# 2892931976/consensus-rs

Measured on AMD Instinct MI355X. Metric: BFT instance-rounds/sec (whole node), N=64 f=21, 1/2/4/8 GPUs; bit-exact, higher is better.
Workload: dtype u64

## Files before the change

### __graft_entry__.py

```python
import os
import subprocess
import sys

ROOT = os.path.dirname(os.path.abspath(__file__))
PKG = os.path.join(ROOT, "consensus-rs_amd")


def _make(path, *targets):
    jobs = str(min(8, os.cpu_count() or 1))
    subprocess.check_call(["make", "-s", "-j", jobs, "-C", path, *targets])


def build() -> None:
    env_arch = os.environ.get("PYTORCH_ROCM_ARCH", "gfx950")
    assert "gfx950" in env_arch, "this framework targets gfx950 only"
    _make(PKG)
    _make(os.path.join(ROOT, "oracle"))
    sys.path.insert(0, os.path.join(ROOT, "tests"))
    import emu_lib
    emu_lib.build()
    import sig_lib
    sig_lib.build()
    import wire_lib
    wire_lib.build()
    import trace_lib
    trace_lib.build()
    import twins_lib
    twins_lib.build()
    import audit_lib
    audit_lib.build()
    import ledger_lib
    ledger_lib.build()
    import archive_lib
    archive_lib.build()
    import accuse_lib
    accuse_lib.build()
    import timeline_lib
    timeline_lib.build()
    import rollcall_lib
    rollcall_lib.build()
    sys.path.insert(0, PKG)
    import bftsim
    from bftsim import runtime
    runtime.lib()
    from bftsim import sig, wire
    sig.lib()
    wire.lib()


def smoke() -> None:
    sys.path.insert(0, PKG)
    sys.path.insert(0, os.path.join(ROOT, "tests"))
    import numpy as np
    import torch
    from bftsim.configs import cfg3
    from bftsim.runtime import Simulator
    import oracle_lib as O
    assert torch.cuda.is_available(), "smoke() needs an MI355X"
    cfg = cfg3(heights=10)
    sim = Simulator(cfg, device=0)
    got = sim.run(0, 4)
    sim.close()
    ref = O.run(cfg, 0, 4)
    for k in ("committed_height", "flags", "ticks", "views", "round", "proposer", "variant",
              "time_tick", "block_hash"):
        if not np.array_equal(got[k], ref[k]):
            raise AssertionError(f"smoke: HIP result differs from the oracle in {k}")
    assert (got["committed_height"] == 10).all()
    print("smoke ok:", int(got["views"].sum()), "instance-rounds bit-exact vs oracle")


if __name__ == "__main__":
    build()
    if len(sys.argv) > 1 and sys.argv[1] == "smoke":
        smoke()
```

### consensus-rs_amd/csrc/bft_common.h

```cpp
#pragma once
#include <stdint.h>

#if defined(__HIPCC__)
#include <hip/hip_runtime.h>
#define BFT_FN __host__ __device__ inline
#else
#define BFT_FN inline
#endif

namespace bft {

struct Params {
    uint32_t n;
    uint32_t seg;
    uint32_t heights;
    uint32_t hcap;
    uint32_t max_ticks;
    uint32_t block_period;
    uint64_t genesis_time;
    uint64_t seed;
    uint32_t thr16;
    uint32_t byz_count;
    uint32_t crash_thr32;
    uint32_t crash_on;
// ... 643 lines not shown
    return (uint32_t)((((uint64_t)hi << 32) | lo) >> (8u * r));
#endif
}
BFT_FN uint32_t splice_blocks(uint32_t len_p, uint32_t len_s) { return (len_p + len_s + 136u) / 136u; }
BFT_FN uint32_t splice_word(const uint32_t* sx, uint32_t r, const uint32_t* pw, uint32_t w, uint32_t nb) {
    uint32_t v = align_bytes(sx[w + 1u], sx[w], r);
    if (w < 2u * PFX_WORDS) v |= pw[w];
    if (w == 34u * nb - 1u) v ^= 0x80000000u;
    return v;
}
BFT_FN uint32_t header_words(uint64_t* wb, const uint32_t prev[8], const uint8_t* addr20, uint64_t seed,
                             uint32_t inst, uint32_t h, uint32_t prop, uint32_t var, uint64_t time) {
    HdrWriter w(wb);
    header_fields(w, prev, addr20, seed, inst, h, prop, var, time);
    return w.finish();
}
BFT_FN uint32_t header_raw(uint64_t* wb, const uint32_t prev[8], const uint8_t* addr20, uint64_t seed,
                           uint32_t inst, uint32_t h, uint32_t prop, uint32_t var, uint64_t time) {
    HdrWriter w(wb);
    header_fields(w, prev, addr20, seed, inst, h, prop, var, time);
    const uint32_t len = 8u * w.wi + w.fill;
    if (w.fill) wb[w.wi] = w.acc;
    return len;
}

BFT_FN void lane_block_hash(uint8_t* buf, const uint32_t prev[8], const uint8_t* addr20, uint64_t seed,
                            uint32_t inst, uint32_t h, uint32_t prop, uint32_t var, uint64_t time,
                            uint32_t out[8]) {
    uint64_t* wb = (uint64_t*)buf;
    const uint32_t nb = header_words(wb, prev, addr20, seed, inst, h, prop, var, time);
    uint64_t a[25];
#pragma unroll
    for (int i = 0; i < 25; ++i) a[i] = 0;
#pragma unroll 1
    for (uint32_t blk = 0; blk < nb; ++blk) {
        const uint64_t* w = wb + 17u * blk;
#pragma unroll
        for (int i = 0; i < 17; ++i) a[i] ^= w[i];
        keccak_f1600(a);
    }
#pragma unroll
    for (int i = 0; i < 4; ++i) { out[2 * i] = (uint32_t)a[i]; out[2 * i + 1] = (uint32_t)(a[i] >> 32); }
}

BFT_FN uint32_t header_prefix_regs(const uint32_t prev[8], const PfxSel* tbl, uint32_t pw[2 * PFX_WORDS]) {
    uint64_t wv[PFX_WORDS];
#pragma unroll
    for (uint32_t k = 0; k < PFX_WORDS; ++k) wv[k] = 0;
    uint64_t acc = 0x2000dc9dull;
    uint32_t fill = 4, wi = 0;
#pragma unroll
    for (uint32_t i = 0; i < 8; ++i) {
        const uint32_t w = prev[i];
        const uint32_t idx = ((((w >> 7) & 0x01010101u) * 0x10204080u) >> 28);
        const PfxSel sel = tbl[idx];
        const uint64_t v = (uint64_t)perm_bytes(0xccccccccu, w, sel.lo) | ((uint64_t)perm_bytes(0xccccccccu, w, sel.hi) << 32);
        const uint32_t n = 4u + (uint32_t)__builtin_popcount(idx);
        const uint32_t sh = 8u * fill, nf = fill + n;
        const uint64_t lo = acc | (v << sh);
#pragma unroll
        for (uint32_t k = (1u + i) / 2u; k <= i; ++k) wv[k] = wi == k ? lo : wv[k];
        const bool full = nf >= 8u;
        acc = full ? (sh ? v >> (64u - sh) : 0ull) : lo;
        wi += full ? 1u : 0u;
        fill = full ? nf - 8u : nf;
    }
#pragma unroll
    for (uint32_t k = 4; k < PFX_WORDS; ++k) wv[k] = wi == k ? acc : wv[k];
#pragma unroll
    for (uint32_t k = 0; k < PFX_WORDS; ++k) { pw[2 * k] = (uint32_t)wv[k]; pw[2 * k + 1] = (uint32_t)(wv[k] >> 32); }
    return 8u * wi + fill;
}

#if !defined(__HIP_DEVICE_COMPILE__)
inline void spliced_block_hash(const uint32_t* sfx, const uint32_t prev[8], uint32_t out[8]) {
    for (int i = 0; i < 8; ++i) out[i] = 0;
    uint32_t buf[SFX_BUF] = {};
    for (uint32_t i = 0; i < SFX_BODY_DW; ++i) buf[SFX_PAD + i] = sfx[i];
    uint64_t pfx[PFX_WORDS + 4], ref[PFX_WORDS];
    PfxSel tbl[16];
    for (uint32_t i = 0; i < 16; ++i) tbl[i] = pfx_sel(i);
    const uint32_t lp = header_prefix_perm(pfx, prev, tbl);
    if (header_prefix(ref, prev) != lp) return;
    for (uint32_t i = 0; i < PFX_WORDS; ++i) if (ref[i] != pfx[i]) return;
    uint32_t pr[2 * PFX_WORDS];
    if (header_prefix_regs(prev, tbl, pr) != lp) return;
    for (uint32_t i = 0; i < PFX_WORDS; ++i) if (pr[2 * i] != (uint32_t)ref[i] || pr[2 * i + 1] != (uint32_t)(ref[i] >> 32)) return;
    uint32_t pw[2 * PFX_WORDS];
    for (uint32_t i = 0; i < PFX_WORDS; ++i) { pw[2 * i] = (uint32_t)pfx[i]; pw[2 * i + 1] = (uint32_t)(pfx[i] >> 32); }
    const uint32_t c = 72u - lp, nb = splice_blocks(lp, sfx[SFX_LEN_DW]);
    const uint32_t* sx = buf + (c >> 2);
    uint64_t a[25] = {};
    for (uint32_t blk = 0; blk < nb; ++blk) {
        for (uint32_t i = 0; i < 17; ++i) {
            const uint32_t w = 34u * blk + 2u * i;
            a[i] ^= (uint64_t)splice_word(sx, c & 3u, pw, w, nb) | ((uint64_t)splice_word(sx, c & 3u, pw, w + 1u, nb) << 32);
        }
        keccak_f1600(a);
    }
    for (int i = 0; i < 4; ++i) { out[2 * i] = (uint32_t)a[i]; out[2 * i + 1] = (uint32_t)(a[i] >> 32); }
}
#endif

template <uint32_t STRIDE = 1>
BFT_FN uint64_t byz_mask64(uint64_t seed, uint32_t inst, uint32_t f, uint8_t* perm) {
    auto at = [&](uint32_t i) -> uint8_t& { return perm[(i >> 2) * 4u * STRIDE + (i & 3u)]; };
    for (uint32_t i = 0; i < 64u; ++i) at(i) = (uint8_t)i;
    uint64_t mask = 0;
    if (f > 64u) f = 64u;
    for (uint32_t i = 0; i < f; ++i) {
        uint32_t w[4];
        philox(seed, inst, i, 0, DOM_BYZ, w);
        const uint32_t j = i + w[0] % (64u - i);
        const uint8_t t = at(i); at(i) = at(j); at(j) = t;
        mask |= 1ull << at(i);
    }
    return mask;
}
constexpr uint32_t SPEC_VALID = 0x80000000u;
BFT_FN bool spec_block64(uint64_t seed, uint32_t inst, uint32_t x, uint64_t byz, uint32_t tip_w0, uint32_t& j,
                         uint32_t& var) {
    j = tip_w0 & 63u;
    uint64_t v1m = 0;
    if ((byz >> j) & 1ull) {
        uint32_t w[4];
        philox(seed, inst, x, 0, DOM_SPLIT, w);
        v1m = ((uint64_t)w[0] | ((uint64_t)w[1] << 32)) & ~(1ull << j);
    }
    const uint64_t hon = ~byz;
    const bool k0 = __builtin_popcountll(byz | (hon & ~v1m)) > 42, k1 = __builtin_popcountll(byz | (hon & v1m)) > 42;
    var = k1 ? 1u : 0u;
    return k0 != k1;
}
BFT_FN uint32_t spec_word(uint32_t j, uint32_t var, uint32_t seed_next) { return SPEC_VALID | j | (var << 8) | (seed_next << 16); }

BFT_FN uint32_t seed_from_hash(const uint8_t* h, uint32_t n, bool le = false) {
    if (le) {
        uint64_t v = 0;
        for (int i = 7; i >= 0; --i) v = (v << 8) | h[i];
        return (uint32_t)(v % n);
    }
    uint64_t be = 0;
    for (int i = 0; i < 8; ++i) be = (be << 8) | h[i];
    uint64_t a = be % n;
    uint64_t t = (0xffffffffffffffffull % n + 1ull) % n;
    return (uint32_t)((a * t) % n);
}
BFT_FN uint32_t seed_from_words(uint32_t w0, uint32_t w1, uint32_t n, bool le) {
    uint8_t hb[8];
    for (int q = 0; q < 4; ++q) { hb[q] = (uint8_t)(w0 >> (8 * q)); hb[4 + q] = (uint8_t)(w1 >> (8 * q)); }
    return seed_from_hash(hb, n, le);
}

}
```

### consensus-rs_amd/csrc/bft_hip.h

```cpp
#pragma once
#include <hip/hip_runtime.h>

#include "../../include/bftsim.h"
#include "bft_common.h"
#include "bft_wave.h"

namespace bft {

struct WaveHip {
    __device__ void init(uint8_t*) {}
    __device__ static uint32_t lane() { return __lane_id(); }
    __device__ static uint64_t ballot(bool p) { return __builtin_amdgcn_ballot_w64(p); }
    __device__ static uint32_t shfl_xor(uint32_t v, int m) { return (uint32_t)__shfl_xor((int)v, m, 64); }
    __device__ static uint32_t shfl(uint32_t v, uint32_t src) { return (uint32_t)__shfl((int)v, (int)src, 64); }
    template <int N> __device__ static uint32_t row_shl(uint32_t v) {
        return (uint32_t)__builtin_amdgcn_mov_dpp((int)v, 0x100 + N, 0xF, 0xF, true);
    }
    template <int N> __device__ static uint32_t row_shr(uint32_t v) {
        return (uint32_t)__builtin_amdgcn_mov_dpp((int)v, 0x110 + N, 0xF, 0xF, true);
    }
    __device__ static uint32_t bperm(uint32_t addr, uint32_t v) { return (uint32_t)__builtin_amdgcn_ds_bpermute((int)addr, (int)v); }
    __device__ static uint32_t pair_swap(uint32_t v) { return (uint32_t)__builtin_amdgcn_mov_dpp((int)v, 0xB1, 0xF, 0xF, false); }
    template <uint32_t N> __device__ static uint32_t rotl_pair(uint32_t mine, uint32_t other) {
        if constexpr (N == 0) return mine;
// ... 60 lines not shown
    __device__ static void gadd64(uint64_t* p, uint64_t v) { atomicAdd((unsigned long long*)p, (unsigned long long)v); }
};

template <int NW>
struct GroupHip {
    uint64_t* slot;
    uint32_t par;
    __device__ void init(uint8_t* p) { slot = (uint64_t*)p; par = 0; }
    __device__ uint32_t lane() const { return threadIdx.x; }
    __device__ uint64_t* cur() const { return slot + par * 4u; }
    __device__ Bits<NW> ballot(bool p) {
        uint64_t b = __ballot(p);
        uint64_t* s = cur();
        if (__lane_id() == 0) s[threadIdx.x >> 6] = b;
        __syncthreads();
        Bits<NW> r;
#pragma unroll
        for (int k = 0; k < NW; ++k) r.w[k] = s[k];
        par ^= 1u;
        return r;
    }
    __device__ uint32_t bcast(uint32_t v, uint32_t j) {
        uint64_t* s = cur();
        if (threadIdx.x == j) s[0] = v;
        __syncthreads();
        uint32_t r = (uint32_t)s[0];
        par ^= 1u;
        return r;
    }
    __device__ uint32_t grp_max(uint32_t v) {
        for (int m = 1; m < 64; m <<= 1) { uint32_t o = (uint32_t)__shfl_xor((int)v, m, 64); v = v > o ? v : o; }
        uint64_t* s = cur();
        if (__lane_id() == 0) s[threadIdx.x >> 6] = v;
        __syncthreads();
        uint32_t r = 0;
#pragma unroll
        for (int k = 0; k < NW; ++k) r = (uint32_t)s[k] > r ? (uint32_t)s[k] : r;
        par ^= 1u;
        return r;
    }
    __device__ uint32_t grp_or(uint32_t v) {
        for (int m = 1; m < 64; m <<= 1) v |= (uint32_t)__shfl_xor((int)v, m, 64);
        uint64_t* s = cur();
        if (__lane_id() == 0) s[threadIdx.x >> 6] = v;
        __syncthreads();
        uint32_t r = 0;
#pragma unroll
        for (int k = 0; k < NW; ++k) r |= (uint32_t)s[k];
        par ^= 1u;
        return r;
    }
    __device__ uint64_t grp_sum64(uint32_t v32) {
        uint64_t v = v32;
        for (int m = 1; m < 64; m <<= 1) {
            uint32_t lo = (uint32_t)__shfl_xor((int)(uint32_t)v, m, 64), hi = (uint32_t)__shfl_xor((int)(uint32_t)(v >> 32), m, 64);
            v += (uint64_t)lo | ((uint64_t)hi << 32);
        }
        uint64_t* s = cur();
        if (__lane_id() == 0) s[threadIdx.x >> 6] = v;
        __syncthreads();
        uint64_t r = 0;
#pragma unroll
        for (int k = 0; k < NW; ++k) r += s[k];
        par ^= 1u;
        return r;
    }
    __device__ void sync() { __syncthreads(); par ^= 1u; }
    __device__ uint64_t* big() const { return slot + 8 + par * 64u; }
    template <int K> __device__ void ballot_k(const bool (&p)[K], Bits<NW> (&out)[K]) {
        static_assert(K * NW <= 64, "batched ballot area");
        uint64_t* s = big();
        uint64_t b[K];
#pragma unroll
        for (int k = 0; k < K; ++k) b[k] = __ballot(p[k]);
        if (__lane_id() == 0) {
#pragma unroll
            for (int k = 0; k < K; ++k) s[k * NW + (threadIdx.x >> 6)] = b[k];
        }
        __syncthreads();
#pragma unroll
        for (int k = 0; k < K; ++k)
#pragma unroll
            for (int w = 0; w < NW; ++w) out[k].w[w] = s[k * NW + w];
        par ^= 1u;
    }
    __device__ uint64_t* summary() const { return slot + 8 + 2u * 64u; }
    template <int K> __device__ void ballot_k_store(const bool (&p)[K], uint64_t* dst) {
        uint64_t b[K];
#pragma unroll
        for (int k = 0; k < K; ++k) b[k] = __ballot(p[k]);
        if (__lane_id() == 0) {
#pragma unroll
            for (int k = 0; k < K; ++k) dst[k * NW + (threadIdx.x >> 6)] = b[k];
        }
        __syncthreads();
        par ^= 1u;
    }
    template <int K> __device__ void gather_k(const bool (&wr)[K], const uint32_t (&v)[K], uint32_t (&out)[K]) {
        static_assert(K <= 128, "batched gather area");
        uint32_t* s = (uint32_t*)big();
#pragma unroll
        for (int k = 0; k < K; ++k)
            if (wr[k]) s[k] = v[k];
        __syncthreads();
#pragma unroll
        for (int k = 0; k < K; ++k) out[k] = s[k];
        par ^= 1u;
    }
    __device__ static uint64_t clock() { return __builtin_amdgcn_s_memtime(); }
    __device__ static uint32_t gload(const uint32_t* p) {
        return __hip_atomic_load(p, __ATOMIC_RELAXED, __HIP_MEMORY_SCOPE_AGENT);
    }
    __device__ static void gstore(uint32_t* p, uint32_t v) {
        __hip_atomic_store(p, v, __ATOMIC_RELAXED, __HIP_MEMORY_SCOPE_AGENT);
    }
    __device__ static void gstore4(uint32_t* p, uint32_t a, uint32_t b, uint32_t c, uint32_t d) {
        *(uint4*)p = make_uint4(a, b, c, d);
    }
    __device__ static void lds_add(uint32_t* p, uint32_t v) { atomicAdd(p, v); }
    __device__ static void gadd64(uint64_t* p, uint64_t v) { atomicAdd((unsigned long long*)p, (unsigned long long)v); }
};

hipError_t launch_general_0_0(uint32_t seg, dim3 grid, size_t lds, hipStream_t s, const Params& p);
hipError_t launch_general_0_1(uint32_t seg, dim3 grid, size_t lds, hipStream_t s, const Params& p);
hipError_t launch_general_1_0(uint32_t seg, dim3 grid, size_t lds, hipStream_t s, const Params& p);
hipError_t launch_general_1_1(uint32_t seg, dim3 grid, size_t lds, hipStream_t s, const Params& p);
inline hipError_t launch_general(bool need_seed, bool ext, uint32_t seg, dim3 grid, size_t lds, hipStream_t s,
                                 const Params& p) {
    if (need_seed) return ext ? launch_general_1_1(seg, grid, lds, s, p) : launch_general_1_0(seg, grid, lds, s, p);
    return ext ? launch_general_0_1(seg, grid, lds, s, p) : launch_general_0_0(seg, grid, lds, s, p);
}
hipError_t launch_fast(dim3 grid, hipStream_t s, const Params& p);
hipError_t launch_hash_suffix(uint32_t n, uint32_t x0, uint32_t rows, uint32_t* sfx, bool loop, hipStream_t s,
                              Params p);
constexpr uint32_t CHAIN_KERNEL_PAIR = 0, CHAIN_KERNEL_WAVE = 1, CHAIN_KERNEL_LANE = 2;
hipError_t launch_hash_chain(uint32_t n, uint32_t x0, uint32_t rows, uint32_t* sfx, uint32_t kind, hipStream_t s,
                             Params p);
constexpr uint32_t CHAIN_MAX_SETS = 32;
struct ChainSets {
    uint32_t count;
    const uint32_t* sfx[CHAIN_MAX_SETS];
    const uint32_t* ch[CHAIN_MAX_SETS];
    uint8_t* hash[CHAIN_MAX_SETS];
    uint32_t first[CHAIN_MAX_SETS];
    uint64_t* byz[CHAIN_MAX_SETS];
    uint32_t* bad[CHAIN_MAX_SETS];
    const uint32_t* rec[CHAIN_MAX_SETS];
    uint32_t* pred[CHAIN_MAX_SETS];
};
constexpr uint32_t CHAIN_RECORDED = 0;
constexpr uint32_t CHAIN_PREDICTED = 1;
constexpr uint32_t CHAIN_REPAIR = 2;
hipError_t launch_hash_chain_batch(uint32_t n, const ChainSets& cs, uint32_t kind, hipStream_t s, Params p);
hipError_t launch_spec_suffix(uint32_t n, const ChainSets& cs, hipStream_t s, const Params& p);
hipError_t launch_spec_verify(uint32_t n, const ChainSets& cs, hipStream_t s, const Params& p);
hipError_t launch_seed_chain(uint32_t n, hipStream_t s, const Params& p);
hipError_t launch_resume(dim3 grid, size_t lds, hipStream_t s, const Params& p);

}
```

### consensus-rs_amd/csrc/bftsim.hip

```cpp
#include <hip/hip_runtime.h>

#include <stdio.h>
#include <stdlib.h>
#include <string.h>

#include <dlfcn.h>
#include <unistd.h>
#include <rccl/rccl.h>
#include <hipcub/hipcub.hpp>

#include <mutex>
#include <string>
#include <utility>
#include <vector>

#include "bft_hip.h"
#include "bft_fast64.h"
#include "bft_crypto.h"
#include "bft_trace.h"
#include "bft_twins.h"
#include "bft_audit.h"
#include "bft_archive.h"
#include "bft_accuse.h"
#include "bft_timeline.h"
// ... 616 lines not shown
    use_set0_scratch(h);
    if (h->n_sets == 0) {
        (void)hipFree(h->d_ch); (void)hipFree(h->d_flags); (void)hipFree(h->d_ticks); (void)hipFree(h->d_views);
        (void)hipFree(h->d_rec); (void)hipFree(h->d_hash);
    }
    for (uint32_t k = 0; k < h->n_sets; ++k) {
        bftsim::RowSet& r = h->sets[k];
        (void)hipFree(r.ch); (void)hipFree(r.flags); (void)hipFree(r.ticks); (void)hipFree(r.views);
        (void)hipFree(r.rec); (void)hipFree(r.hash); (void)hipFree(r.sfx); (void)hipFree(r.spec);
        (void)hipFree(r.byz); (void)hipFree(r.bad); (void)hipFree(r.pred);
        if (k > 0) {
            (void)hipFree(r.hist); (void)hipFree(r.rcs); (void)hipFree(r.backlog); (void)hipFree(r.resume);
            (void)hipFree(r.save); (void)hipFree(r.resume_q);
        }
        r.ch = r.flags = r.ticks = nullptr; r.views = nullptr; r.rec = nullptr; r.hash = nullptr; r.sfx = nullptr;
        r.spec = nullptr; r.byz = nullptr; r.bad = nullptr; r.pred = nullptr;
        r.hist = nullptr; r.rcs = r.backlog = r.resume = r.save = r.resume_q = nullptr;
    }

    (void)hipFree(h->d_trace); (void)hipFree(h->d_tips); (void)hipFree(h->d_rcs);
    h->d_rcs = nullptr;
    (void)hipFree(h->d_backlog);
    h->d_backlog = nullptr;
    (void)hipFree(h->d_mlog); (void)hipFree(h->d_mlog_n);
    h->d_mlog = nullptr; h->d_mlog_n = nullptr;
    (void)hipFree(h->d_vsnap); (void)hipFree(h->d_votes); (void)hipFree(h->d_vsig); (void)hipFree(h->d_vhas);
    h->d_vsnap = nullptr; h->d_votes = nullptr; h->d_vsig = nullptr; h->d_vhas = nullptr; h->vsig_n = 0;
    h->backlog_bytes = 0;
    (void)hipFree(h->d_resume); (void)hipFree(h->d_save); (void)hipFree(h->d_resume_q);
    h->d_resume = nullptr; h->d_save = nullptr; h->d_resume_q = nullptr;
    for (uint32_t k = 0; k < bftsim::MAX_SETS; ++k) h->sets[k].busy = false;
    h->n_sets = 0;
    h->cur_set = 0;
    h->d_ch = h->d_flags = h->d_ticks = nullptr; h->d_views = nullptr;
    h->d_rec = nullptr; h->d_hash = nullptr; h->d_trace = nullptr; h->d_tips = nullptr;
    h->cap_inst = 0;
    h->n_req = 0;
    h->last_n = 0;
    h->last_first = 0;
}

static int flush_batch(bftsim* h, bool final = false);
static int sync_all(bftsim* h) {
    HIPCHECK(h, hipSetDevice(h->device));
    if (int rc = flush_batch(h, true)) return rc;
    HIPCHECK(h, hipStreamSynchronize(h->last_stream));
    for (uint32_t k = 0; k < bftsim::MAX_CS; ++k)
        if (h->cs[k]) HIPCHECK(h, hipStreamSynchronize(h->cs[k]));
    for (uint32_t k = 0; k < bftsim::MAX_HS; ++k)
        if (h->hstr[k]) HIPCHECK(h, hipStreamSynchronize(h->hstr[k]));
    return BFTSIM_OK;
}

#ifdef BFT_STAMPS
static uint64_t* g_stamps = nullptr;
static uint64_t g_stamp_waves = 0;
#endif

namespace {
struct Rccl {
    ncclResult_t (*get_id)(ncclUniqueId*) = nullptr;
    ncclResult_t (*init_rank)(ncclComm_t*, int, ncclUniqueId, int) = nullptr;
    ncclResult_t (*all_reduce)(const void*, void*, size_t, ncclDataType_t, ncclRedOp_t, ncclComm_t,
                               hipStream_t) = nullptr;
    ncclResult_t (*destroy)(ncclComm_t) = nullptr;
    const char* (*err)(ncclResult_t) = nullptr;
    bool ok = false;
    std::string why;
};
Rccl& rccl() {
    static Rccl r;
    static std::once_flag once;
    std::call_once(once, [] {
        void* lib = dlopen("librccl.so.1", RTLD_NOW | RTLD_GLOBAL);
        if (!lib) lib = dlopen("/opt/rocm/lib/librccl.so.1", RTLD_NOW | RTLD_GLOBAL);
        if (!lib) { r.why = std::string("dlopen librccl.so.1: ") + dlerror(); return; }
        r.get_id = (decltype(r.get_id))dlsym(lib, "ncclGetUniqueId");
        r.init_rank = (decltype(r.init_rank))dlsym(lib, "ncclCommInitRank");
        r.all_reduce = (decltype(r.all_reduce))dlsym(lib, "ncclAllReduce");
        r.destroy = (decltype(r.destroy))dlsym(lib, "ncclCommDestroy");
        r.err = (decltype(r.err))dlsym(lib, "ncclGetErrorString");
        r.ok = r.get_id && r.init_rank && r.all_reduce && r.destroy && r.err;
        if (!r.ok) r.why = "librccl.so.1 lacks an entry point";
    });
    return r;
}
struct StdoutToStderr {
    int saved;
    StdoutToStderr() {
        fflush(stdout);
        saved = dup(1);
        if (saved >= 0) dup2(2, 1);
    }
    ~StdoutToStderr() {
        fflush(stdout);
        if (saved >= 0) { dup2(saved, 1); close(saved); }
    }
};
void comm_destroy(ncclComm_t c) {
    if (rccl().ok) (void)rccl().destroy(c);
}

struct SigApi {
    int (*create)(int, void**) = nullptr;
    void (*destroy)(void*) = nullptr;
    const char* (*last_error)(const void*) = nullptr;
    int (*secret_to_address)(void*, const uint8_t*, uint64_t, uint8_t*, uint8_t*, uint8_t*, void*) = nullptr;
    int (*sign)(void*, const uint8_t*, const uint32_t*, const uint8_t*, uint64_t, uint8_t*, uint8_t*, void*) = nullptr;
    int (*recover)(void*, const uint8_t*, const uint8_t*, uint64_t, uint8_t*, uint8_t*, uint8_t*, void*) = nullptr;
    bool ok = false;
    std::string why;
};
void sig_api_anchor() {}
SigApi& sig_api() {
    static SigApi a;
    static std::once_flag once;
    std::call_once(once, [] {
        Dl_info di;
        std::string path = "libbftsig.so";
        if (dladdr((void*)&sig_api_anchor, &di) && di.dli_fname) {
            std::string self = di.dli_fname;
            size_t k = self.rfind('/');
            if (k != std::string::npos) path = self.substr(0, k + 1) + "libbftsig.so";
        }
        void* lib = dlopen(path.c_str(), RTLD_NOW | RTLD_GLOBAL);
        if (!lib) { a.why = std::string("dlopen ") + path + ": " + dlerror(); return; }
        a.create = (decltype(a.create))dlsym(lib, "bftsig_create");
        a.destroy = (decltype(a.destroy))dlsym(lib, "bftsig_destroy");
        a.last_error = (decltype(a.last_error))dlsym(lib, "bftsig_last_error");
        a.secret_to_address = (decltype(a.secret_to_address))dlsym(lib, "bftsig_secret_to_address");
        a.sign = (decltype(a.sign))dlsym(lib, "bftsig_sign");
        a.recover = (decltype(a.recover))dlsym(lib, "bftsig_recover");
        a.ok = a.create && a.destroy && a.last_error && a.secret_to_address && a.sign && a.recover;
        if (!a.ok) a.why = path + " lacks an entry point";
    });
    return a;
}
}

extern "C" {

#ifdef BFT_STAMPS
int bftsim_debug_stamps(uint64_t* out, uint32_t cap) {
    if (!out || cap == 0) return bft::NSTAMP;
    std::vector<uint64_t> v(g_stamp_waves * bft::NSTAMP);
    if (hipDeviceSynchronize() != hipSuccess) return -2;
    if (hipMemcpy(v.data(), g_stamps, v.size() * 8, hipMemcpyDeviceToHost) != hipSuccess) return -2;
    const uint32_t m = cap < (uint32_t)bft::NSTAMP ? cap : (uint32_t)bft::NSTAMP;
    for (uint32_t k = 0; k < m; ++k) out[k] = 0;
    for (uint64_t w = 0; w < g_stamp_waves; ++w)
        for (uint32_t k = 0; k < m; ++k) out[k] += v[w * bft::NSTAMP + k];
    return bft::NSTAMP;
}
#endif

uint32_t bftsim_two_thirds_majority(uint32_t n) { return (2u * n) / 3u; }
uint32_t bftsim_seed_from_hash(const uint8_t hash[32], uint32_t n) { return n ? bft::seed_from_hash(hash, n) : 0; }
uint32_t bftsim_seed_from_hash_order(const uint8_t hash[32], uint32_t n, uint32_t order) {
    return n ? bft::seed_from_hash(hash, n, order == BFTSIM_SEED_LE) : 0;
}
uint32_t bftsim_calc_proposer(const uint8_t prev_hash[32], uint32_t n, uint64_t round) {
    if (n == 0) return 0;
    return (uint32_t)(((uint64_t)bft::seed_from_hash(prev_hash, n) + round % n) % n);
}
void bftsim_keccak256(const uint8_t* data, size_t len, uint8_t out[32]) { host_keccak(data, len, out); }
void bftsim_genesis_hash(const bftsim_config* cfg, uint8_t out[32]) { host_genesis_hash(cfg, out); }
int bftsim_check_message(uint32_t code, uint64_t msg_height, uint64_t core_height, uint32_t state) {
    if (code < 1 || code > 4 || state < 1 || state > 4 || msg_height >= (1ull << 32) || core_height >= (1ull << 32))
        return BFTSIM_EINVAL;
    return bft::check_message_class((int)code, (uint32_t)msg_height, (uint32_t)core_height, state);
}
int bftsim_view_cmp(uint64_t h1, uint64_t r1, uint64_t h2, uint64_t r2) {
    if (h1 != h2) return h1 < h2 ? -1 : 1;
    if (r1 != r2) return r1 < r2 ? -1 : 1;
    return 0;
}

const char* bftsim_last_error(bftsim_t* h) { return h ? h->err.c_str() : "null handle"; }

int bftsim_create(const bftsim_config* cfg, int hip_device, bftsim_t** out) {
    if (!cfg || !out) return BFTSIM_EINVAL;
    *out = nullptr;
    if (cfg->n < 1 || cfg->n > 256) return BFTSIM_EUNSUPPORTED;
    if (cfg->heights < 1 || cfg->heights > (1u << 20) || cfg->max_ticks < 1 || cfg->max_ticks > (1u << 28) ||
        !cfg->addresses || cfg->phase_cap < 1 || cfg->phase_cap > 255 || cfg->block_period < 1)
        return BFTSIM_EINVAL;
    for (uint32_t i = 1; i < cfg->n; ++i)
        if (memcmp(cfg->addresses + 20 * (i - 1), cfg->addresses + 20 * i, 20) >= 0) return BFTSIM_EINVAL;
    if (cfg->seed_byte_order > BFTSIM_SEED_LE || cfg->header_encoding != BFTSIM_ENC_RMP_COMPACT ||
        cfg->backlog_mode > BFTSIM_BACKLOG_REPLAY || cfg->reserved != 0)
        return BFTSIM_EINVAL;
    bftsim* h = new bftsim();
    h->cfg = *cfg;
    h->addresses.assign(cfg->addresses, cfg->addresses + 20 * cfg->n);
    h->cfg.addresses = h->addresses.data();
    h->device = hip_device;
    host_genesis_hash(&h->cfg, h->genesis_hash);
    h->genesis_seed = bft::seed_from_hash(h->genesis_hash, cfg->n, cfg->seed_byte_order == BFTSIM_SEED_LE);
    h->seg = bft::segment_size(cfg->n);
    h->hcap = cfg->heights + 64;
    *out = h;
    hipError_t e = hipSetDevice(hip_device);
    if (e != hipSuccess) return fail(h, BFTSIM_EHIP, std::string("hipSetDevice: ") + hipGetErrorString(e));
    HIPCHECK(h, hipMalloc(&h->d_addr, 20 * cfg->n));
    HIPCHECK(h, hipMemcpy(h->d_addr, h->addresses.data(), 20 * cfg->n, hipMemcpyHostToDevice));
    HIPCHECK(h, hipMalloc(&h->d_ghash, 32));
    HIPCHECK(h, hipMemcpy(h->d_ghash, h->genesis_hash, 32, hipMemcpyHostToDevice));
    HIPCHECK(h, hipMalloc(&h->d_stats, 16 * sizeof(unsigned long long)));
    HIPCHECK(h, hipMalloc(&h->d_hist, bft::HIST_BINS * sizeof(uint64_t)));
    for (uint32_t i = 0; i < bftsim::RING; ++i) {
        HIPCHECK(h, hipEventCreate(&h->ring[i].c0)); HIPCHECK(h, hipEventCreate(&h->ring[i].c1));
        HIPCHECK(h, hipEventCreate(&h->ring[i].h0)); HIPCHECK(h, hipEventCreate(&h->ring[i].h1));
        HIPCHECK(h, hipEventCreateWithFlags(&h->ring[i].sx, hipEventDisableTiming));
    }
    for (uint32_t i = 0; i < bftsim::MAX_SETS; ++i)
        HIPCHECK(h, hipEventCreateWithFlags(&h->sets[i].done, hipEventDisableTiming));
    return BFTSIM_OK;
}

void bftsim_destroy(bftsim_t* h) {
    if (!h) return;
    (void)hipSetDevice(h->device);
    free_bufs(h);
    (void)hipFree(h->d_addr); (void)hipFree(h->d_ghash); (void)hipFree(h->d_stats); (void)hipFree(h->d_hist);
    (void)hipFree(h->d_red);
    (void)hipFree(h->d_evict);
    (void)hipFree(h->d_keys);
    if (h->comm) comm_destroy(h->comm);
    if (h->sig) sig_api().destroy(h->sig);
    for (uint32_t i = 0; i < bftsim::RING; ++i) {
        if (h->ring[i].c0) (void)hipEventDestroy(h->ring[i].c0);
        if (h->ring[i].c1) (void)hipEventDestroy(h->ring[i].c1);
        if (h->ring[i].h0) (void)hipEventDestroy(h->ring[i].h0);
        if (h->ring[i].h1) (void)hipEventDestroy(h->ring[i].h1);
        if (h->ring[i].sx) (void)hipEventDestroy(h->ring[i].sx);
    }
    for (uint32_t i = 0; i < bftsim::MAX_SETS; ++i) {
        if (h->sets[i].done) (void)hipEventDestroy(h->sets[i].done);
        h->sets[i].batch_done = nullptr;
        if (h->sets[i].entry) (void)hipEventDestroy(h->sets[i].entry);
        if (h->sets[i].hint) (void)hipHostFree(h->sets[i].hint);
    }
    for (uint32_t i = 0; i < bftsim::BATCH_EVS; ++i)
        if (h->batch_ev[i]) (void)hipEventDestroy(h->batch_ev[i]);
    for (uint32_t i = 0; i < bftsim::MAX_CS; ++i)
        if (h->cs[i]) (void)hipStreamDestroy(h->cs[i]);
    for (uint32_t i = 0; i < bftsim::MAX_HS; ++i)
        if (h->hstr[i]) (void)hipStreamDestroy(h->hstr[i]);
    delete h;
}

static bft::Params make_params(bftsim* h, uint64_t first, uint64_t n);

int bftsim_prepare(bftsim_t* h, uint64_t n) {
    if (!h || n == 0 || n > (1ull << 31)) return fail(h, BFTSIM_EINVAL, "bad instance count");
    HIPCHECK(h, hipSetDevice(h->device));
    trace_drop(h);
    if (n <= h->cap_inst) { h->n_req = n; return BFTSIM_OK; }
    if (h->last_n) if (int rc = sync_all(h)) return rc;
    free_bufs(h);
    HIPCHECK(h, hipMalloc(&h->d_ch, n * 4));
    HIPCHECK(h, hipMalloc(&h->d_flags, n * 4));
    HIPCHECK(h, hipMalloc(&h->d_ticks, n * 4));
    HIPCHECK(h, hipMalloc(&h->d_views, n * 8));
    HIPCHECK(h, hipMalloc(&h->d_rec, n * h->hcap * 16));
    HIPCHECK(h, hipMalloc(&h->d_hash, n * h->hcap * 32));
    HIPCHECK(h, hipMalloc(&h->d_tips, n * 32));
    {
        uint64_t per_block = h->seg > 64 ? 1 : 64 / h->seg;
        uint64_t blocks = (n + per_block - 1) / per_block;
        HIPCHECK(h, hipMalloc(&h->d_rcs, blocks * bft::rcs_words(h->seg, h->rcs_k) * 4));
        if (h->crypto) {
            HIPCHECK(h, hipMalloc(&h->d_mlog, n * (uint64_t)h->mlog_cap * bft::MLOG_WORDS * 4));
            HIPCHECK(h, hipMalloc(&h->d_mlog_n, n * 4));
            HIPCHECK(h, hipMalloc(&h->d_vsnap, n * (uint64_t)h->seg * 8 * 4));
            HIPCHECK(h, hipMalloc(&h->d_votes, n * (uint64_t)h->hcap * 8 * 4));
        }
        if (h->cfg.backlog_mode == BFTSIM_BACKLOG_REPLAY) {
            h->backlog_bytes = blocks * bft::backlog_words(h->seg) * 4;
            HIPCHECK(h, hipMalloc(&h->d_backlog, h->backlog_bytes));
        }
    }
    if (h->seg == 64 && h->cfg.n == 64) {
        HIPCHECK(h, hipMalloc(&h->d_resume, n * 4));
        HIPCHECK(h, hipMalloc(&h->d_resume_q, (n + 2) * 4));
        HIPCHECK(h, hipMalloc(&h->d_save, (uint64_t)bft::SAVE_WORDS * n * 64 * 4));
    }
    h->sets[0].ch = h->d_ch; h->sets[0].flags = h->d_flags; h->sets[0].ticks = h->d_ticks;
    h->sets[0].views = h->d_views; h->sets[0].rec = h->d_rec; h->sets[0].hash = h->d_hash;
    h->sets[0].hist = h->d_hist; h->sets[0].rcs = h->d_rcs; h->sets[0].backlog = h->d_backlog;
    h->sets[0].resume = h->d_resume; h->sets[0].save = h->d_save; h->sets[0].resume_q = h->d_resume_q;
    h->n_sets = 1;
    const char* tst = getenv("BFTSIM_TESTING");
    const bool testing = tst && strcmp(tst, "1") == 0;
    auto knob = [&](const char* name, uint32_t& v, uint32_t lo, uint32_t hi) {
        const char* e = getenv(name);
        if (!testing || !e) return false;
        const uint32_t x = (uint32_t)atoi(e);
        v = x < lo ? lo : x > hi ? hi : x;
        return true;
    };
    auto knob64 = [&](const char* name, uint64_t& v) {
        const char* e = getenv(name);
        if (!testing || !e) return false;
        v = strtoull(e, nullptr, 10);
        return true;
// ... 2030 lines not shown
```

### consensus-rs_amd/csrc/kern_fast.hip

```cpp
#include "bft_hip.h"
#include "bft_fast64.h"

namespace bft {

#ifndef BFT_FAST_WAVES_PER_SIMD
#define BFT_FAST_WAVES_PER_SIMD 4
#endif
#ifndef BFT_FAST_LOSSLESS_WAVES_PER_SIMD
#define BFT_FAST_LOSSLESS_WAVES_PER_SIMD 4
#endif
#ifndef BFT_FAST_SEEDED_WAVES_PER_SIMD
#define BFT_FAST_SEEDED_WAVES_PER_SIMD 4
#endif
template <bool LOSSY, bool SEEDED>
__global__ __launch_bounds__(64, SEEDED ? BFT_FAST_SEEDED_WAVES_PER_SIMD
                                        : LOSSY ? BFT_FAST_WAVES_PER_SIMD : BFT_FAST_LOSSLESS_WAVES_PER_SIMD)
void bft_consensus_fast_kernel(Params p) {
    extern __shared__ uint8_t lds[];
#ifndef BFT_CONSENSUS_PRIO
#define BFT_CONSENSUS_PRIO 2
#endif
    __builtin_amdgcn_s_setprio(BFT_CONSENSUS_PRIO);
    Fast64<WaveHip, LOSSY, SEEDED> sim(p, lds, blockIdx.x);
    sim.run();
// ... 219 lines not shown

#if defined(__HIP_DEVICE_COMPILE__)
#ifndef BFT_LANE_UNROLL
#define BFT_LANE_UNROLL 24
#endif
__device__ inline void keccak_f1600_lane(uint32_t L[25], uint32_t H[25]) {
#pragma unroll BFT_LANE_UNROLL
    for (int rnd = 0; rnd < 24; ++rnd) {
        uint32_t cl[5], ch[5], rl[5], rh[5], bl[25], bh[25];
#pragma unroll
        for (int x = 0; x < 5; ++x) {
            cl[x] = xor3_32(xor3_32(L[x], L[x + 5], L[x + 10]), L[x + 15], L[x + 20]);
            ch[x] = xor3_32(xor3_32(H[x], H[x + 5], H[x + 10]), H[x + 15], H[x + 20]);
        }
#pragma unroll
        for (int x = 0; x < 5; ++x) rotl_halves<1>(cl[(x + 1) % 5], ch[(x + 1) % 5], rl[x], rh[x]);
#define BFT_RHO_L(i, n, j) rotl_halves<n>(xor3_32(L[i], cl[((i) % 5 + 4) % 5], rl[(i) % 5]), \
                                          xor3_32(H[i], ch[((i) % 5 + 4) % 5], rh[(i) % 5]), bl[j], bh[j]);
        BFT_RHO_L(0, 0, 0) BFT_RHO_L(1, 1, 10) BFT_RHO_L(2, 62, 20) BFT_RHO_L(3, 28, 5) BFT_RHO_L(4, 27, 15)
        BFT_RHO_L(5, 36, 16) BFT_RHO_L(6, 44, 1) BFT_RHO_L(7, 6, 11) BFT_RHO_L(8, 55, 21) BFT_RHO_L(9, 20, 6)
        BFT_RHO_L(10, 3, 7) BFT_RHO_L(11, 10, 17) BFT_RHO_L(12, 43, 2) BFT_RHO_L(13, 25, 12) BFT_RHO_L(14, 39, 22)
        BFT_RHO_L(15, 41, 23) BFT_RHO_L(16, 45, 8) BFT_RHO_L(17, 15, 18) BFT_RHO_L(18, 21, 3) BFT_RHO_L(19, 8, 13)
        BFT_RHO_L(20, 18, 14) BFT_RHO_L(21, 2, 24) BFT_RHO_L(22, 61, 9) BFT_RHO_L(23, 56, 19) BFT_RHO_L(24, 14, 4)
#undef BFT_RHO_L
#pragma unroll
        for (int y = 0; y < 5; ++y)
#pragma unroll
            for (int x = 0; x < 5; ++x) {
                L[5 * y + x] = bl[5 * y + x] ^ (~bl[5 * y + (x + 1) % 5] & bl[5 * y + (x + 2) % 5]);
                H[5 * y + x] = bh[5 * y + x] ^ (~bh[5 * y + (x + 1) % 5] & bh[5 * y + (x + 2) % 5]);
            }
        L[0] ^= KECCAK_RC_LO[rnd];
        H[0] ^= KECCAK_RC_HI[rnd];
    }
}
#endif

constexpr uint32_t SFX_LDS_DW = 56;
static_assert(SFX_LDS_DW * 4u >= 213u && SFX_LDS_DW <= SFX_BODY_DW && SFX_LDS_DW % 2u == 0u, "inline suffix column");
#if defined(__HIP_DEVICE_COMPILE__)
template <bool INLINE>
__device__ inline void lane_chain(const Params& p, const ChainSets& cs, uint32_t k, uint32_t il, const PfxSel* ptbl,
                                  uint32_t* sl) {
    const uint32_t n = p.n_instances;
    const uint32_t K = p.sfx_rows, x0 = p.sfx_x0;
    uint32_t x1 = x0 + K - 1u, xs = x0;
    if (p.chain_mode != CHAIN_PREDICTED) {
        const uint32_t ch = cs.ch[k][il];
        x1 = ch < x1 ? ch : x1;
        if (p.chain_mode == CHAIN_REPAIR) {
            const uint32_t b = cs.bad[k][il];
            xs = b > x0 ? b : x0;
        }
    }
    if (x1 < xs) return;
    uint8_t* const hash = cs.hash[k];
    const uint32_t* ph = (const uint32_t*)(xs == 1u ? p.genesis_hash : hash + ((uint64_t)il * p.rows + xs - 1u) * 32);
    uint32_t prev[8];
#pragma unroll
    for (int i = 0; i < 8; ++i) prev[i] = ph[i];
    const char* const sbase = (const char*)cs.sfx[k];
    const uint32_t n4 = 4u * n;
    const uint32_t* const rec = cs.rec[k] + (uint64_t)il * p.rows * 4u;
    const bool predicted = INLINE && p.chain_mode == CHAIN_PREDICTED;
    uint64_t byz = 0;
    if (predicted) {
        byz = byz_mask64<64>(p.seed, cs.first[k] + il, p.byz_count, (uint8_t*)sl);
        cs.bad[k][il] = 0xffffffffu;
    }
    uint32_t* const pred = predicted ? cs.pred[k] + (uint64_t)il * p.heights : nullptr;
    for (uint32_t x = xs; x <= x1; ++x) {
        const uint32_t rowoff = 4u * il + (x - x0) * SFX_DEV_DW * n4;
        uint32_t len_s;
        if constexpr (INLINE) {
            uint32_t prop, var, tick;
            if (p.chain_mode == CHAIN_PREDICTED) {
                const bool ok = spec_block64(p.seed, cs.first[k] + il, x, byz, 0u, prop, var);
                pred[x - 1u] = ok ? SPEC_VALID | prop | (var << 16) : 0u;
                if (!ok) break;
                tick = x - 1u;
            } else {
                const uint4 row = *(const uint4*)(rec + 4u * x);
                prop = row.y & 0xffffu;
                var = (row.y >> 16) & 1u;
                tick = row.z;
            }
            HdrWriter w(sl, 64u);
            header_suffix_fields(w, p.addresses + 20u * prop, p.seed, cs.first[k] + il, x, prop, var,
                                 p.genesis_time + (uint64_t)p.block_period * ((uint64_t)tick + 1ull));
            len_s = 8u * w.wi + w.fill;
            w.store(w.wi++, w.acc | (0x01ull << (8u * w.fill)));
            while (w.wi < SFX_LDS_DW / 2u) w.store(w.wi++, 0);
        } else {
            len_s = *(const uint32_t*)(sbase + rowoff + SFX_DEV_LEN_DW * n4);
        }
        if (len_s == 0u) break;
        uint32_t pw[2 * PFX_WORDS];
        const uint32_t len_p = header_prefix_regs(prev, ptbl, pw);
        const uint32_t c = 72u - len_p, r = c & 3u, nb = splice_blocks(len_p, len_s);
        const int j0 = (int)(c >> 2) - (int)SFX_PAD;
        auto G = [&](uint32_t jj) -> uint32_t {
            if constexpr (INLINE) return sl[64u * jj];
            else return *(const uint32_t*)(sbase + rowoff + __umul24(jj, n4));
        };
        constexpr int BODY = INLINE ? (int)SFX_LDS_DW : (int)SFX_BODY_DW;
        auto S = [&](int j) -> uint32_t {
            const uint32_t v = G((uint32_t)(j < 0 ? 0 : j > BODY - 1 ? BODY - 1 : j));
            return ((j >= 0) & (j < BODY)) ? v : 0u;
        };
        uint32_t L[25], H[25];
#pragma unroll
        for (int i = 0; i < 25; ++i) {
            L[i] = i < (int)PFX_WORDS ? pw[2 * i] : 0u;
            H[i] = i < (int)PFX_WORDS ? pw[2 * i + 1] : 0u;
        }
        for (uint32_t blk = 0; blk < nb; ++blk) {
            uint32_t d[35];
            if (blk == 0u) {
#pragma unroll
                for (int i = 0; i < 17; ++i) d[i] = S(j0 + i);
                if constexpr (INLINE) {
#pragma unroll
                    for (int i = 17; i < 35; ++i) d[i] = G((uint32_t)(j0 + i));
                } else {
                    uint32_t vo = rowoff + __umul24((uint32_t)(j0 + 17), n4);
#pragma unroll
                    for (int i = 17; i < 35; ++i, vo += n4) d[i] = *(const uint32_t*)(sbase + vo);
                }
#pragma unroll
                for (int i = 0; i < 34; ++i) d[i] = align_bytes(d[i + 1], d[i], r);
            } else {
#pragma unroll
                for (int i = 0; i < 35; ++i) d[i] = S(j0 + 34 * (int)blk + i);
#pragma unroll
                for (int i = 0; i < 34; ++i) d[i] = align_bytes(d[i + 1], d[i], r);
            }
#pragma unroll
            for (int i = 0; i < 17; ++i) { L[i] ^= d[2 * i]; H[i] ^= d[2 * i + 1]; }
            if (blk + 1u == nb) H[16] ^= 0x80000000u;
            keccak_f1600_lane(L, H);
        }
        uint32_t* dst = (uint32_t*)(hash + ((uint64_t)il * p.rows + x) * 32);
#pragma unroll
        for (int i = 0; i < 4; ++i) { prev[2 * i] = L[i]; prev[2 * i + 1] = H[i]; }
        *(uint4*)dst = make_uint4(prev[0], prev[1], prev[2], prev[3]);
        *(uint4*)(dst + 4) = make_uint4(prev[4], prev[5], prev[6], prev[7]);
    }
}
#endif
#ifndef BFT_LANE_WAVES_PER_SIMD
#define BFT_LANE_WAVES_PER_SIMD 4
#endif

template <bool INLINE>
__global__ __launch_bounds__(64, INLINE ? BFT_LANE_WAVES_PER_SIMD : 3) void bft_hash_chain_lane_kernel(Params p, ChainSets cs) {
#if defined(__HIP_DEVICE_COMPILE__)
    set_prio(p.chain_prio);
    __shared__ PfxSel ptbl[16];
    extern __shared__ uint32_t sfx_lds[];
    if (threadIdx.x < 16) ptbl[threadIdx.x] = PFX_TBL[threadIdx.x];
    __syncthreads();
    const uint32_t bps = (p.n_instances + 63u) / 64u, tasks = cs.count * bps;
    for (uint32_t t = blockIdx.x; t < tasks; t += gridDim.x) {
        const uint32_t k = t / bps, il = (t % bps) * 64u + threadIdx.x;
        if (il < p.n_instances)
            lane_chain<INLINE>(p, cs, k, il, ptbl, INLINE ? sfx_lds + threadIdx.x : nullptr);
    }
#endif
}
static hipError_t launch_lane(uint32_t tasks, const ChainSets& cs, hipStream_t s, const Params& p) {
    const uint32_t g = p.chain_grid && p.chain_grid < tasks ? p.chain_grid : tasks;
    if (p.chain_inline)
        hipLaunchKernelGGL(bft_hash_chain_lane_kernel<true>, dim3(g), dim3(64), (size_t)SFX_LDS_DW * 64u * 4u, s, p, cs);
    else hipLaunchKernelGGL(bft_hash_chain_lane_kernel<false>, dim3(g), dim3(64), 0, s, p, cs);
    return hipGetLastError();
}

__global__ __launch_bounds__(256) void bft_spec_byz_kernel(Params p, ChainSets cs) {
    set_prio(p.chain_prio);
    __shared__ uint8_t perm[256 * 64];
    const uint32_t n = p.n_instances, bpl = (n + 255u) / 256u, k = blockIdx.x / bpl;
    const uint32_t il = (blockIdx.x % bpl) * 256u + threadIdx.x;
    if (il >= n) return;
    cs.byz[k][il] = byz_mask64(p.seed, cs.first[k] + il, p.byz_count, perm + 64u * threadIdx.x);
    cs.bad[k][il] = 0xffffffffu;
}
__device__ inline uint64_t spec_time(const Params& p, uint32_t tick) {
    return p.genesis_time + (uint64_t)p.block_period * ((uint64_t)tick + 1ull);
}
__global__ __launch_bounds__(256) void bft_spec_suffix_kernel(Params p, ChainSets cs) {
    set_prio(p.chain_prio);
    const uint32_t n = p.n_instances, H = p.heights;
    const uint32_t bpl = (uint32_t)(((uint64_t)n * H + 255u) / 256u), k = blockIdx.x / bpl;
    const uint32_t t = (blockIdx.x % bpl) * 256u + threadIdx.x;
    const uint32_t j = t / n, il = t - j * n;
    if (j >= H) return;
    const uint32_t x = j + 1u, inst = cs.first[k] + il;
    uint32_t* row = const_cast<uint32_t*>(cs.sfx[k]) + (uint64_t)j * SFX_DEV_DW * n + il;
    uint32_t prop, var;
    if (!spec_block64(p.seed, inst, x, cs.byz[k][il], 0u, prop, var)) {
        row[(uint64_t)SFX_DEV_LEN_DW * n] = 0u;
        cs.pred[k][(uint64_t)il * H + j] = 0u;
        return;
    }
    cs.pred[k][(uint64_t)il * H + j] = SPEC_VALID | prop | (var << 16);
    header_suffix_strided(row, n, p.addresses + 20u * prop, p.seed, inst, x, prop, var, spec_time(p, x - 1u));
}
__global__ __launch_bounds__(256) void bft_spec_verify_kernel(Params p, ChainSets cs) {
    const uint32_t n = p.n_instances, H = p.heights;
    const uint32_t bpl = (uint32_t)(((uint64_t)n * H + 255u) / 256u), k = blockIdx.x / bpl;
    const uint32_t t = (blockIdx.x % bpl) * 256u + threadIdx.x;
    const uint32_t il = t / H, x = t - il * H + 1u;
    if (il >= n) return;
    if (x > cs.ch[k][il]) return;
    const uint4 row = *(const uint4*)(cs.rec[k] + ((uint64_t)il * p.rows + x) * 4);
    const uint32_t pw = cs.pred[k][(uint64_t)il * H + x - 1u], inst = cs.first[k] + il;
    if (((pw & SPEC_VALID) != 0u) & ((row.y & 0x1ffffu) == (pw & 0x1ffffu)) & (row.z + 1u == x)) return;
    const uint32_t rp = row.y & 0xffffu, rv = (row.y >> 16) & 1u;
    header_suffix_strided(const_cast<uint32_t*>(cs.sfx[k]) + (uint64_t)(x - 1u) * SFX_DEV_DW * n + il, n,
                          p.addresses + 20u * rp, p.seed, inst, x, rp, rv, spec_time(p, row.z));
    atomicMin(&cs.bad[k][il], x);
}
hipError_t launch_spec_suffix(uint32_t n, const ChainSets& cs, hipStream_t s, const Params& p) {
    if (cs.count < 1 || cs.count > CHAIN_MAX_SETS || p.n_instances != n) return hipErrorInvalidValue;
    hipLaunchKernelGGL(bft_spec_byz_kernel, dim3(cs.count * ((n + 255u) / 256u)), dim3(256), 0, s, p, cs);
    const uint32_t bpl = (uint32_t)(((uint64_t)n * p.heights + 255u) / 256u);
    hipLaunchKernelGGL(bft_spec_suffix_kernel, dim3(cs.count * bpl), dim3(256), 0, s, p, cs);
    return hipGetLastError();
}
hipError_t launch_spec_verify(uint32_t n, const ChainSets& cs, hipStream_t s, const Params& p) {
    if (cs.count < 1 || cs.count > CHAIN_MAX_SETS || p.n_instances != n) return hipErrorInvalidValue;
    const uint32_t bpl = (uint32_t)(((uint64_t)n * p.heights + 255u) / 256u);
    hipLaunchKernelGGL(bft_spec_verify_kernel, dim3(cs.count * bpl), dim3(256), 0, s, p, cs);
    return hipGetLastError();
}

__global__ __launch_bounds__(CHAIN_PAIR_BLOCK) void bft_seed_chain_kernel(Params p) {
#if defined(__HIP_DEVICE_COMPILE__)
    __shared__ __attribute__((aligned(16))) uint32_t sbuf[32 * CHAIN_SB];
    __shared__ __attribute__((aligned(16))) uint64_t pbuf[CHAIN_PB_SLOTS * (PFX_WORDS + 4)];
    __shared__ PfxSel ptbl[16];
    __shared__ uint32_t slen[32];
    if (threadIdx.x < 16) ptbl[threadIdx.x] = PFX_TBL[threadIdx.x];
    __syncthreads();
    const uint32_t odd = threadIdx.x & 1u, pair = threadIdx.x >> 1;
    const uint32_t il = blockIdx.x * 32u + pair;
    if (il >= p.n_instances) return;
    const uint32_t n = p.n_instances, inst = p.first_instance + il;
    uint32_t* sb = sbuf + pair * CHAIN_SB;
    const uint64_t byz = byz_mask64(p.seed, inst, p.byz_count, (uint8_t*)(sb + SFX_PAD) + 64u * odd);
    __syncthreads();
    for (uint32_t i = odd; i < SFX_PAD; i += 2u) sb[i] = 0;
    for (uint32_t i = SFX_PAD + SFX_BODY_DW + odd; i < CHAIN_SB; i += 2u) sb[i] = 0;
    const uint8_t* ph = p.genesis_hash;
    uint32_t prev[8];
    for (int i = 0; i < 8; ++i)
        prev[i] = (uint32_t)ph[4 * i] | ((uint32_t)ph[4 * i + 1] << 8) | ((uint32_t)ph[4 * i + 2] << 16) |
                  ((uint32_t)ph[4 * i + 3] << 24);
    uint64_t* pb = pbuf + (BFT_CHAIN_COMPACT ? pair : threadIdx.x) * (PFX_WORDS + 4);
    const uint32_t* pw = (const uint32_t*)pb + odd;
    for (uint32_t x = 1; x <= p.heights; ++x) {
        uint32_t j, var;
        if (!spec_block64(p.seed, inst, x, byz, prev[0], j, var)) {
            if (!odd) p.spec[(uint64_t)x * n + il] = 0u;
            break;
        }
        if (!odd) {
            HdrWriter w(sb + SFX_PAD, 1u);
            header_suffix_fields(w, p.addresses + 20u * j, p.seed, inst, x, j, var,
                                 p.genesis_time + (uint64_t)p.block_period * (uint64_t)x);
            slen[pair] = 8u * w.wi + w.fill;
            w.store(w.wi++, w.acc | (0x01ull << (8u * w.fill)));
            while (w.wi < SFX_BODY_DW / 2u) w.store(w.wi++, 0);
        }
        const uint32_t len_p = header_prefix_perm(pb, prev, ptbl);
        __syncthreads();
        pair_header_hash(sb, pw, odd, len_p, slen[pair], prev, (uint32_t*)(p.hash + ((uint64_t)il * p.rows + x) * 32));
        if (!odd) p.spec[(uint64_t)x * n + il] = spec_word(j, var, seed_from_words(prev[0], prev[1], 64u, true));
        __syncthreads();
    }
#endif
}
hipError_t launch_seed_chain(uint32_t n, hipStream_t s, const Params& p) {
    hipLaunchKernelGGL(bft_seed_chain_kernel, dim3((n + 31u) / 32u), dim3(CHAIN_PAIR_BLOCK), 0, s, p);
    return hipGetLastError();
}

__global__ __launch_bounds__(64) void bft_hash_chain_wave_kernel(Params p, ChainSets cs) {
    __shared__ __attribute__((aligned(16))) uint32_t sb[SFX_BUF];
    __shared__ __attribute__((aligned(16))) uint32_t pf[KW_PFX_DW];
    set_prio(p.chain_prio);
    const uint32_t lane = threadIdx.x;
    const uint32_t bps = 8u * ((p.n_instances + 7u) / 8u), k = blockIdx.x / bps, b = blockIdx.x % bps;
    p.sfx = const_cast<uint32_t*>(cs.sfx[k]);
    p.committed_height = const_cast<uint32_t*>(cs.ch[k]);
    p.hash = cs.hash[k];
    const uint32_t per = bps >> 3;
    const uint32_t il = (b & 7u) * per + (b >> 3);
    if (il >= p.n_instances) return;
    const uint32_t K = p.sfx_rows, x0 = p.sfx_x0;
    const uint32_t ch = p.committed_height[il];
    const uint32_t x1 = ch < x0 + K - 1u ? ch : x0 + K - 1u;
    if (x1 < x0) return;
    const uint32_t* ph = (const uint32_t*)(x0 == 1u ? p.genesis_hash : p.hash + ((uint64_t)il * p.rows + x0 - 1u) * 32);
    const uint32_t a_prev = lane < 8u ? ph[lane] : 0u;
    WaveHip wv;
    kw50_chain(wv, lane, sb, pf, p.sfx + il, (uint64_t)SFX_DEV_DW * p.n_instances, p.n_instances, a_prev,
               x1 - x0 + 1u, (uint32_t*)(p.hash + ((uint64_t)il * p.rows + x0) * 32));
}

hipError_t launch_hash_suffix(uint32_t n, uint32_t x0, uint32_t rows, uint32_t* sfx, bool loop, hipStream_t s,
                              Params p) {
    p.sfx = sfx;
    p.sfx_rows = rows;
    p.sfx_x0 = x0;
    if (loop) hipLaunchKernelGGL(bft_hash_suffix_loop_kernel, dim3((n + 255u) / 256u), dim3(256), 0, s, p);
    else hipLaunchKernelGGL(bft_hash_suffix_kernel, dim3((uint32_t)(((uint64_t)n * rows + 255u) / 256u)), dim3(256), 0, s, p);
    return hipGetLastError();
}
hipError_t launch_hash_chain(uint32_t n, uint32_t x0, uint32_t rows, uint32_t* sfx, uint32_t kind, hipStream_t s,
                             Params p) {
    p.sfx = sfx;
    p.sfx_rows = rows;
    p.sfx_x0 = x0;
    ChainSets cs{};
    cs.count = 1; cs.sfx[0] = sfx; cs.ch[0] = p.committed_height; cs.hash[0] = p.hash;
    cs.rec[0] = p.rec; cs.first[0] = p.first_instance;
    if (kind == CHAIN_KERNEL_LANE && 4ull * n >= (1ull << 24)) kind = CHAIN_KERNEL_PAIR;
// ... 20 lines not shown
```

Measured before the change: 3.520 billion.

## Pack four hash-chain lane waves per workgroup and add census instrumentation

The lane hash-chain kernel now runs several 64-lane waves per workgroup, four for predicted and repair chains and one for recorded chains. Tasks are spread across waves and workgroups by a new helper, and each wave gets its own LDS suffix slice. This is meant to cut per-workgroup launch and scheduling overhead and change how chain work lands on CUs, at the cost of more LDS per workgroup and possibly lower occupancy. A census recorder that logs per-task timing and hardware ids is also added, compiled only under BFT_STAMPS, and the build now also makes the stamps target.

```diff
diff --git a/__graft_entry__.py b/__graft_entry__.py
--- a/__graft_entry__.py
+++ b/__graft_entry__.py
@@ -14,7 +14,7 @@
 def build() -> None:
     env_arch = os.environ.get("PYTORCH_ROCM_ARCH", "gfx950")
     assert "gfx950" in env_arch, "this framework targets gfx950 only"
-    _make(PKG)
+    _make(PKG, "all", "stamps")
     _make(os.path.join(ROOT, "oracle"))
     sys.path.insert(0, os.path.join(ROOT, "tests"))
     import emu_lib
@@ -39,6 +39,8 @@
     timeline_lib.build()
     import rollcall_lib
     rollcall_lib.build()
+    import place_lib
+    place_lib.build()
     sys.path.insert(0, PKG)
     import bftsim
     from bftsim import runtime
diff --git a/consensus-rs_amd/csrc/bft_common.h b/consensus-rs_amd/csrc/bft_common.h
--- a/consensus-rs_amd/csrc/bft_common.h
+++ b/consensus-rs_amd/csrc/bft_common.h
@@ -819,4 +819,18 @@
     return seed_from_hash(hb, n, le);
 }
 
-}
+constexpr uint32_t LANE_WG_WAVES = 4;
+BFT_FN uint32_t lane_chain_wgs(uint32_t grid_waves, uint32_t tasks, uint32_t waves) {
+    const uint32_t g = grid_waves && grid_waves < tasks ? grid_waves : tasks;
+    return (g + waves - 1u) / waves;
+}
+BFT_FN bool lane_chain_task(uint32_t wg, uint32_t wave, uint32_t wgs, uint32_t waves, uint32_t it, uint32_t bps,
+                            uint32_t tasks, uint32_t& k, uint32_t& first) {
+    const uint32_t t = waves * (it * wgs + wg) + wave;
+    if (t >= tasks) return false;
+    k = t / bps;
+    first = (t % bps) * 64u;
+    return true;
+}
+
+}
diff --git a/consensus-rs_amd/csrc/bft_hip.h b/consensus-rs_amd/csrc/bft_hip.h
--- a/consensus-rs_amd/csrc/bft_hip.h
+++ b/consensus-rs_amd/csrc/bft_hip.h
@@ -236,6 +236,9 @@
 constexpr uint32_t CHAIN_PREDICTED = 1;
 constexpr uint32_t CHAIN_REPAIR = 2;
 hipError_t launch_hash_chain_batch(uint32_t n, const ChainSets& cs, uint32_t kind, hipStream_t s, Params p);
+#ifdef BFT_STAMPS
+int census_fetch(uint64_t* out, uint32_t cap);
+#endif
 hipError_t launch_spec_suffix(uint32_t n, const ChainSets& cs, hipStream_t s, const Params& p);
 hipError_t launch_spec_verify(uint32_t n, const ChainSets& cs, hipStream_t s, const Params& p);
 hipError_t launch_seed_chain(uint32_t n, hipStream_t s, const Params& p);
diff --git a/consensus-rs_amd/csrc/bftsim.hip b/consensus-rs_amd/csrc/bftsim.hip
--- a/consensus-rs_amd/csrc/bftsim.hip
+++ b/consensus-rs_amd/csrc/bftsim.hip
@@ -792,6 +792,7 @@
         for (uint32_t k = 0; k < m; ++k) out[k] += v[w * bft::NSTAMP + k];
     return bft::NSTAMP;
 }
+int bftsim_debug_census(uint64_t* out, uint32_t cap) { return bft::census_fetch(out, cap); }
 #endif
 
 uint32_t bftsim_two_thirds_majority(uint32_t n) { return (2u * n) / 3u; }
diff --git a/consensus-rs_amd/csrc/kern_fast.hip b/consensus-rs_amd/csrc/kern_fast.hip
--- a/consensus-rs_amd/csrc/kern_fast.hip
+++ b/consensus-rs_amd/csrc/kern_fast.hip
@@ -395,28 +395,79 @@
 #define BFT_LANE_WAVES_PER_SIMD 4
 #endif
 
-template <bool INLINE>
-__global__ __launch_bounds__(64, INLINE ? BFT_LANE_WAVES_PER_SIMD : 3) void bft_hash_chain_lane_kernel(Params p, ChainSets cs) {
+#ifdef BFT_STAMPS
+struct CensusRec { uint32_t k , task, hw_id, xcc_id; uint64_t t0, t1; };
+constexpr uint32_t CENSUS_CAP = 1u << 16;
+static CensusRec* g_census = nullptr;
+static uint32_t g_census_used = 0;
+#define BFT_CENSUS_PARAM , CensusRec* census
+#define BFT_CENSUS_ARG , census_take(tasks)
+static CensusRec* census_take(uint32_t tasks) {
+    if (!g_census && hipMalloc(&g_census, sizeof(CensusRec) * (size_t)CENSUS_CAP) != hipSuccess) return nullptr;
+    if (tasks > CENSUS_CAP - g_census_used) return nullptr;
+    CensusRec* r = g_census + g_census_used;
+    g_census_used += tasks;
+    return r;
+}
+int census_fetch(uint64_t* out, uint32_t cap) {
+    if (hipDeviceSynchronize() != hipSuccess) return -2;
+    const uint32_t n = g_census_used < cap ? g_census_used : cap;
+    static_assert(sizeof(CensusRec) == 32, "four 64-bit words");
+    if (n && hipMemcpy(out, g_census, sizeof(CensusRec) * (size_t)n, hipMemcpyDeviceToHost) != hipSuccess) return -2;
+    const int total = (int)g_census_used;
+    g_census_used = 0;
+    return total;
+}
+#else
+#define BFT_CENSUS_PARAM
+#define BFT_CENSUS_ARG
+#endif
+
+template <bool INLINE, uint32_t WAVES>
+__global__ __launch_bounds__(64 * WAVES, INLINE ? BFT_LANE_WAVES_PER_SIMD : 3)
+void bft_hash_chain_lane_kernel(Params p, ChainSets cs BFT_CENSUS_PARAM) {
 #if defined(__HIP_DEVICE_COMPILE__)
     set_prio(p.chain_prio);
     __shared__ PfxSel ptbl[16];
     extern __shared__ uint32_t sfx_lds[];
     if (threadIdx.x < 16) ptbl[threadIdx.x] = PFX_TBL[threadIdx.x];
     __syncthreads();
+    const uint32_t wave = __builtin_amdgcn_readfirstlane(threadIdx.x >> 6);
+    const uint32_t lane = __builtin_amdgcn_mbcnt_hi(~0u, __builtin_amdgcn_mbcnt_lo(~0u, 0u));
     const uint32_t bps = (p.n_instances + 63u) / 64u, tasks = cs.count * bps;
-    for (uint32_t t = blockIdx.x; t < tasks; t += gridDim.x) {
-        const uint32_t k = t / bps, il = (t % bps) * 64u + threadIdx.x;
-        if (il < p.n_instances)
-            lane_chain<INLINE>(p, cs, k, il, ptbl, INLINE ? sfx_lds + threadIdx.x : nullptr);
-    }
-#endif
+    uint32_t* const sl = INLINE ? sfx_lds + wave * (SFX_LDS_DW * 64u) + lane : nullptr;
+    uint32_t k, first;
+    for (uint32_t it = 0; lane_chain_task(blockIdx.x, wave, gridDim.x, WAVES, it, bps, tasks, k, first); ++it) {
+#ifdef BFT_STAMPS
+        const uint64_t t0 = wall_clock64();
+#endif
+        if (first + lane < p.n_instances) lane_chain<INLINE>(p, cs, k, first + lane, ptbl, sl);
+#ifdef BFT_STAMPS
+        if (census && lane == 0u) {
+            CensusRec r;
+            r.k = k | (p.chain_mode << 16);
+            r.task = k * bps + first / 64u;
+            r.hw_id = __builtin_amdgcn_s_getreg(4 | (31 << 11));
+            r.xcc_id = __builtin_amdgcn_s_getreg(20 | (3 << 11));
+            r.t0 = t0;
+            r.t1 = wall_clock64();
+            census[r.task] = r;
+        }
+#endif
+    }
+#endif
+}
+template <uint32_t WAVES>
+static hipError_t launch_lane_wg(uint32_t tasks, const ChainSets& cs, hipStream_t s, const Params& p) {
+    const uint32_t g = lane_chain_wgs(p.chain_grid, tasks, WAVES);
+    if (p.chain_inline)
+        hipLaunchKernelGGL((bft_hash_chain_lane_kernel<true, WAVES>), dim3(g), dim3(64u * WAVES),
+                           (size_t)WAVES * SFX_LDS_DW * 64u * 4u, s, p, cs BFT_CENSUS_ARG);
+    else hipLaunchKernelGGL((bft_hash_chain_lane_kernel<false, WAVES>), dim3(g), dim3(64u * WAVES), 0, s, p, cs BFT_CENSUS_ARG);
+    return hipGetLastError();
 }
 static hipError_t launch_lane(uint32_t tasks, const ChainSets& cs, hipStream_t s, const Params& p) {
-    const uint32_t g = p.chain_grid && p.chain_grid < tasks ? p.chain_grid : tasks;
-    if (p.chain_inline)
-        hipLaunchKernelGGL(bft_hash_chain_lane_kernel<true>, dim3(g), dim3(64), (size_t)SFX_LDS_DW * 64u * 4u, s, p, cs);
-    else hipLaunchKernelGGL(bft_hash_chain_lane_kernel<false>, dim3(g), dim3(64), 0, s, p, cs);
-    return hipGetLastError();
+    return p.chain_mode == CHAIN_RECORDED ? launch_lane_wg<1>(tasks, cs, s, p) : launch_lane_wg<LANE_WG_WAVES>(tasks, cs, s, p);
 }
 
 __global__ __launch_bounds__(256) void bft_spec_byz_kernel(Params p, ChainSets cs) {
```

Result: slower. 3.468 billion (-1.5%).
